# AnimatePortrait/AnimatePortrait

Measured on AMD Instinct MI355X. Metric: generator frames/sec @256x256 bs=16, higher is better.
Workload: dtype f32 (fp32 tensors; wide convs multiply fp32-class on the bf16 pipe: operands as bf16 head + tail, 3 products of 16-bit significands per multiply, ~2^-17 relative per product, fp32 accumulate); 1 GPU; Module2 generator resnet_9blocks_rcatland32_full_ifw fwd-only, ngf=64, bs=16/GPU, 256x256, fp32 (BASELINE configs[1]); global_batch=16, parallelism=dp1 (frame batches sharded, no collective), weights=random init N(0,0.02), seed 1234

## Files before the change

### animateportrait_amd/autograd.py

```python
import collections

import torch

from . import ops
from .ops import Feat, ConvSpec, ACT_NONE, ACT_RELU, ACT_LRELU, ACT_TANH, PAD_ZERO, PAD_REFLECT, W_OIHW, W_IOHW


_DIRECT = 0


class direct_param_grads:

    def __enter__(self):
        global _DIRECT
        _DIRECT += 1

    def __exit__(self, *exc):
        global _DIRECT
        _DIRECT -= 1
        return False


class Tape:
    def __init__(self):
# ... 159 lines not shown

def conv_backward(tape, layer, srcs, out, norm, act):
    contribs = tape.take(out)
    if not contribs:
        return
    plan = _backward_plan(tape, layer, srcs, out, norm, act, contribs)
    gfeat, gt, strip, db = _backward_norm(tape, plan, layer, out, act, contribs)
    _backward_weight(tape, plan, layer, srcs, gfeat, gt)
    _backward_bias(tape, layer, norm, gfeat, db)
    _backward_data(tape, plan, layer, srcs, gfeat, strip)


def _backward_norm(tape, plan, layer, out, act, contribs):
    if plan.norm_route == 'split':
        return ops.instnorm_bwd_split(ops._split_contribs(contribs), out, plan.gt_dims, plan.want_xs, plan.want_strip) + (None,)
    if out.data.dtype != torch.float32:
        out = Feat(out.data.float(), out._mean, out._rstd, out.act)
        contribs = [(g.float() if g.dtype != torch.float32 else g, pd) for g, pd in contribs]
    db = None
    if plan.norm_route == 'instnorm':
        dy = ops.instnorm_bwd(contribs, out, out_bf16=plan.dy16)
    elif plan.norm_route == 'act_bias':
        dy, db = ops.act_bwd_bias(contribs, out.data, act, tape.slot(layer.bias))
    else:
        dy = ops.act_bwd(contribs, out.data, act)
    gfeat = Feat(dy)
    if plan.wgrad_operand == 'g_xs_presplit':
        ops.presplit(gfeat, layer.spec.precision)
    return gfeat, None, None, db


def _backward_weight(tape, plan, layer, srcs, gfeat, gt):
    if plan.wgrad_route is None:
        return
    s = layer.spec
    if s.transposed:
        dw = ops.wgrad(s.k, 2, s.pad, PAD_ZERO, srcs[0], [gfeat], layer.weight.shape, precision=s.precision,
                       out=tape.slot(layer.weight), route=plan.wgrad_route)
    else:
        g_xs = gfeat.xs if plan.wgrad_operand in ('g_xs_from_split', 'g_xs_presplit') else None
        dw = ops.wgrad(s.k, s.stride, s.pad, s.pad_mode, gfeat, srcs, layer.weight.shape, precision=s.precision,
                       out=tape.slot(layer.weight), g_t=gt, g_xs=g_xs, route=plan.wgrad_route)
    tape.add_param(layer.weight, dw)


def _backward_bias(tape, layer, norm, gfeat, db):
    if not layer.bias.requires_grad:
        return
    slot = tape.slot(layer.bias)
    if norm:
        tape.add_param(layer.bias, slot if slot is not None else torch.zeros_like(layer.bias))
    else:
        tape.add_param(layer.bias, db if db is not None else ops.bias_grad(gfeat.data, out=slot))


def _backward_data(tape, plan, layer, srcs, gfeat, strip):
    s = layer.spec
    c0 = 0
    for i, (f, c, route) in enumerate(zip(srcs, s.cin_segments, plan.dgrad)):
        if route is not None and route[0] == 'final_k7':
            tape.add(f, ops.final_dgrad_k7(gfeat, layer.weight), route[1])
        elif route is not None and route[0] == 'head':
            tape.add(f, ops.head_dgrad(gfeat, layer.weight, f.data.shape[2], f.data.shape[3]), route[1])
        elif route is not None:
            spec, _ = _dgrad_spec(layer, c)
            w = layer.weight.detach()
            if len(srcs) > 1:
                w = w[c0:c0 + c] if s.transposed else w[:, c0:c0 + c]
            packed = layer.packed_dgrad(i, spec, w)
            if route[0] == 'strip':
                packed_t = layer.packed_dgrad((i, 'T'), spec, w.transpose(2, 3))
                g = ops.conv2d_dgrad_strip(spec, gfeat, packed, packed_t, strip, out_bf16=f.data.dtype == torch.bfloat16)
            else:
                g = ops.conv2d(spec, [gfeat], packed, None).data
            tape.add(f, g, route[1])
        c0 += c


def conv_forward(tape, layer, srcs, norm_act=None, act=ACT_NONE, out_octet=False, raw16=False):
    if not isinstance(srcs, (list, tuple)):
        srcs = [srcs]
    raw16 = (raw16 and tape is not None and norm_act is not None and ops.BF16_RAW and ops.DEFAULT_PRECISION == ops.PRECISION_BF16 and
             layer.spec.precision == ops.PRECISION_BF16)
    out = layer.run(srcs, norm_act=norm_act, act=act, out_octet=out_octet and tape is None, out_bf16=raw16)
    if tape is not None:
        tape.track(out)
        norm = norm_act is not None
        tape.steps.append(lambda: conv_backward(tape, layer, srcs, out, norm, act))
    return out


def _reduced(tape, f):
    contribs = tape.take(f)
    if not contribs:
        return None
    g1, pad, g2 = ops._split_contribs(contribs)
    return g1 if (pad == 0 and g2 is None) else ops.fold_add(g1, pad, g2)


def materialize_forward(tape, f, residual=None, consumer=None):
    keep = tape is not None or (consumer is not None and not consumer.stages_split(f.data.shape))
    out = ops.materialize(f, residual=residual, keep_fp32=keep)
    if tape is not None:
        tape.track(out)

        def bwd():
            g = _reduced(tape, out)
            if g is None:
                return
            tape.add(f, g, 0)
            if residual is not None:
                tape.add(residual, g, 0)
        tape.steps.append(bwd)
    return out


def warp_forward(tape, f, motion, flow, ifmask, level, consumer=None):
    n, _, h, w = f.data.shape
    emit_xs = consumer is not None and ops.takes_split(consumer.spec, n, h, w)
    s2d = emit_xs and len(consumer.spec.cin_segments) == 1 and ops.s2d_eligible(consumer.spec, h, w)
    out = ops.warp_concat(f, motion, flow, ifmask, level, emit_xs=emit_xs, keep_fp32=tape is not None or not emit_xs, s2d=s2d)
    if tape is not None:
        tape.track(out)

        def bwd():
            g = _reduced(tape, out)
            if g is None or not tape.tracked(f):
                return
            tape.add(f, ops.warp_concat_bwd(g, motion, flow, ifmask, level), 0)
        tape.steps.append(bwd)
    return out


def batch_split_forward(tape, f, b):
    l1, l2 = f.batch_slice(0, b), f.batch_slice(b, 2 * b)
    if tape is not None:
        tape.track(l1)
        tape.track(l2)

        def bwd():
            tape.add(f, torch.cat([_reduced(tape, l1), _reduced(tape, l2)], 0), 0)
        tape.steps.append(bwd)
    return l1, l2


def _weights_stamp(params):
    return tuple(ops.weight_key(p) for p in params)


class _NetFn(torch.autograd.Function):
    @staticmethod
    def forward(ctx, net, n_inputs, input_needs_grad, *tensors):
        inputs, params = tensors[:n_inputs], tensors[n_inputs:]
        tape = Tape()
        with torch.no_grad():
            out = net._run(tape, input_needs_grad, *inputs)
        ctx.tape, ctx.net, ctx.out_feat = tape, net, out
        ctx.n_inputs, ctx.params = n_inputs, params
        ctx.stamp = _weights_stamp(params)
        ctx.in_feat = getattr(net, '_last_input_feat', None)
        return out.data

    @staticmethod
    def backward(ctx, gout):
        tape = ctx.tape
        if tape is None:
            raise RuntimeError('animateportrait_amd: backward through this network a second time: the layer tape is '
# ... 34 lines not shown
```

### animateportrait_amd/networks.py

```python
import functools

import torch
import torch.nn as nn
from torch.optim import lr_scheduler

from . import ops
from .autograd import (conv_forward, materialize_forward, warp_forward, batch_split_forward,
                       generator_apply, discriminator_apply)
from .ops import (Feat, ConvSpec, ACT_NONE, ACT_RELU, ACT_LRELU, ACT_TANH, PAD_ZERO, PAD_REFLECT,
                  W_OIHW, W_IOHW)

GENERATOR_NAMES = ('resnet_9blocks_rcatland32_full_ifw', 'resnet_style2_9blocks')
_REFERENCE_ONLY_G = (
    'resnet_9blocks', 'resnet_9blocks_rcatland', 'resnet_9blocks_rcatland3',
    'resnet_9blocks_rcatland32', 'resnet_10blocks_rcatland32', 'resnet_9blocks_rcatland4',
    'resnet_9blocks_rcatland32_fw', 'resnet_9blocks_rcatland32_fw2', 'resnet_9blocks_rcatland32_ifw',
    'resnet_9blocks_rcatland32_ifw_single2', 'resnet_9blocks_rcatland32_full_ifw_colorcoded',
    'resnet_9blocks_rcatland32_full_ifw2', 'resnet_9blocks_rcatland32_full_ifw_single',
    'resnet_9blocks_rcatland32_full_ifw_single2', 'resnet_9blocks_rcatland32_full_ifw_single3', 'regressor',
    'combiner', 'resnet_9blocks_rcatland2', 'resnet_6blocks', 'unet_128', 'unet_256')


class ConvLayer(nn.Module):

    def __init__(self, cin_segments, cout, k, stride=1, pad=0, pad_mode=PAD_ZERO, transposed=False,
                 output_padding=0):
        super().__init__()
        cin = sum(cin_segments)
        shape = (cin, cout, k, k) if transposed else (cout, cin, k, k)
        self.weight = nn.Parameter(torch.empty(shape, dtype=torch.float32))
        self.bias = nn.Parameter(torch.zeros(cout, dtype=torch.float32))
        self.spec = ConvSpec(cin_segments, cout, k, stride, pad, pad_mode, transposed, output_padding,
                             W_IOHW if transposed else W_OIHW)
        self._slots = {}
        self._rows_spec = None
        self._s2d_spec = None

    def _packed(self, slot_id, spec, view):
        slot = ops.packed_slot(spec, self.weight, view, self._slots.get(slot_id))
        self._slots[slot_id] = slot
        return slot.buf

    def packed_dgrad(self, seg, spec, view):
        return self._packed(('dgrad', seg), spec, ops.WeightView(view))

    def packed(self):
        return self._packed('fwd', self.spec, ops.WeightView(self.weight.detach()))

    def run(self, srcs, norm_act=None, act=ACT_NONE, out_octet=False, out_bf16=False):
        if not isinstance(srcs, (list, tuple)):
            srcs = [srcs]
        spec, packed = self.spec, None
        if norm_act is None and ops.conv_d0_ok(spec, srcs, act):
            return ops.conv_d0(srcs[0], self.weight, self.bias.detach(), act)
        if ops.stem_rows_eligible(spec) and not srcs[0].is_split_only:
            spec, packed = self.rows_spec(), self.packed_rows()
            srcs = [ops.presplit_rows(srcs[0], self.spec.k, self.spec.pad, self.spec.pad_mode)]
        elif (srcs[0].s2d is not None or not srcs[0].is_split_only) and ops.s2d_eligible(spec, *srcs[0].data.shape[2:]):
            spec, packed = self.s2d_spec(), self.packed_s2d()
            if srcs[0].s2d is None:
                srcs[0].s2d = ops.presplit_s2d(srcs[0])
            srcs = [srcs[0].s2d]
        if packed is None:
            packed = self.packed()
        if norm_act is None:
            return ops.conv2d(spec, srcs, packed, self.bias.detach(), act=act, out_octet=out_octet)
        return ops.conv2d(spec, srcs, packed, None, want_stats=True, out_act=norm_act, out_octet=out_octet,
                          out_bf16=out_bf16 and spec is self.spec)

    def stages_split(self, shape):
        n, _, h, w = shape
        if ops.stem_rows_eligible(self.spec) or ops.s2d_eligible(self.spec, h, w):
            return False
        return ops.takes_split(self.spec, n, h, w)

    def s2d_spec(self):
        if self._s2d_spec is None:
            self._s2d_spec = ops.s2d_spec(self.spec)
        return self._s2d_spec

    def packed_s2d(self):
        return self._packed('s2d', self.s2d_spec(), ops.WeightView(self.weight.detach(), s2d_c=self.spec.cin_segments[0]))

    def rows_spec(self):
        if self._rows_spec is None:
            self._rows_spec = ops.stem_rows_spec(self.spec)
        return self._rows_spec

    def packed_rows(self):
        return self._packed('rows', self.rows_spec(), ops.WeightView(self.weight.detach(), rows_c=self.spec.cin_segments[0]))


def _seq(**children):
    return nn.ModuleDict({k.lstrip('_'): v for k, v in children.items()})


class ResnetBlock(nn.Module):

    def __init__(self, dim):
        super().__init__()
        self.conv_block = _seq(_1=ConvLayer([dim], dim, 3, 1, 1, PAD_REFLECT),
                               _5=ConvLayer([dim], dim, 3, 1, 1, PAD_REFLECT))

    def run(self, x, tape=None, consumer=None):
        c1, c5 = self.conv_block['1'], self.conv_block['5']
        dim = c1.spec.cout
        keep = consumer is not None and not consumer.stages_split(x.data.shape)
        y = conv_forward(tape, c1, x, norm_act=ACT_RELU, raw16=True, out_octet=tape is None and ops.trunk_octet_ok(dim))
        y = conv_forward(tape, c5, y, norm_act=ACT_NONE, raw16=True,
                         out_octet=tape is None and ops.trunk_octet_ok(dim, residual=x, keep_fp32=keep))
        return materialize_forward(tape, y, residual=x, consumer=consumer)


class ResnetBlock2(nn.Module):

    def __init__(self, segs, dim_out):
        super().__init__()
        self.conv_block = _seq(_1=ConvLayer(segs, dim_out, 3, 1, 1, PAD_REFLECT),
                               _5=ConvLayer([dim_out], dim_out, 3, 1, 1, PAD_REFLECT))
        self.shortcut = _seq(_0=ConvLayer(segs, dim_out, 3, 1, 1, PAD_ZERO))

    def run(self, srcs, tape=None, consumer=None):
        c1, c5, sc = self.conv_block['1'], self.conv_block['5'], self.shortcut['0']
        y = conv_forward(tape, c1, srcs, norm_act=ACT_RELU, raw16=True, out_octet=tape is None and ops.trunk_octet_ok(c1.spec.cout))
        y = conv_forward(tape, c5, y, norm_act=ACT_NONE, raw16=True)
        s = conv_forward(tape, sc, srcs, norm_act=ACT_NONE)
        return materialize_forward(tape, y, residual=s, consumer=consumer)


class ResnetConditionTriGenerator32_full_ifw(nn.Module):

    def __init__(self, input_nc, output_nc, ngf=64, norm='instance', use_dropout=False, n_blocks=9,
                 padding_type='reflect', div=3, disp=1):
        super().__init__()
        if norm != 'instance':
            raise NotImplementedError('normalization layer [%s] is not available on the HIP path' % norm)
        if use_dropout:
            raise NotImplementedError('dropout is not available on the HIP path (the model sets no_dropout)')
        if padding_type != 'reflect':
            raise NotImplementedError('padding [%s] is not implemented' % padding_type)
        assert n_blocks >= 0
        self.n_blocks, self.div, self.disp = n_blocks, div, disp
        self.input_nc, self.output_nc, self.ngf = input_nc, output_nc, ngf
        h = ngf // 2
        con_dim = 16
        dim = ngf * 4
        self.model_tri_merge = ConvLayer([ngf * 4, ngf * 4, ngf * 4], dim, 3, 1, 1)
        self.model_tri00 = _seq(_1=ConvLayer([input_nc], h, 7, 1, 3, PAD_REFLECT))
        self.model_tri01 = _seq(_0=ConvLayer([ngf], ngf * 2, 3, 2, 1))
        self.model_tri02 = _seq(_0=ConvLayer([ngf * 2], ngf * 4, 3, 2, 1))
        self.model_tri10 = _seq(_1=ConvLayer([input_nc], ngf, 7, 1, 3, PAD_REFLECT))
        self.model_tri11 = _seq(_0=ConvLayer([ngf], ngf, 3, 2, 1))
        self.model_tri12 = _seq(_0=ConvLayer([ngf * 2], ngf * 4, 3, 2, 1))
        self.model_tri20 = _seq(_1=ConvLayer([input_nc], ngf, 7, 1, 3, PAD_REFLECT))
        self.model_tri21 = _seq(_0=ConvLayer([ngf], ngf * 2, 3, 2, 1))
        self.model_tri22 = _seq(_0=ConvLayer([ngf * 2], ngf * 2, 3, 2, 1))
        blocks = {}
        for i in range(n_blocks):
            if (i + disp) % div == 0:
                blocks[str(i)] = ResnetBlock2([dim, con_dim, con_dim], dim)
            else:
                blocks[str(i)] = ResnetBlock(dim)
        self.model2 = nn.ModuleDict(blocks)
        self.model3 = _seq(_0=ConvLayer([ngf * 4], ngf * 2, 3, 2, 1, transposed=True, output_padding=1),
                           _3=ConvLayer([ngf * 2], ngf, 3, 2, 1, transposed=True, output_padding=1),
# ... 292 lines not shown
```

### animateportrait_amd/ops.py

```python
import collections
import ctypes
import os

import torch

from . import _capi as C
from ._capi import ACT_NONE, ACT_RELU, ACT_LRELU, ACT_TANH, PAD_ZERO, PAD_REFLECT, W_OIHW, W_IOHW

EPS = 1e-5

WEIGHTS_EPOCH = 0


def weight_key(w):
    owner = getattr(w, '_flat_owner', None)
    return (w._version, w.data_ptr(), WEIGHTS_EPOCH, owner.epoch if owner is not None else 0)

PRECISION_FP32, PRECISION_BF16X3, PRECISION_BF16 = 0, 1, 2
PRECISION_BY_NAME = {'fp32': PRECISION_FP32, 'bf16x3': PRECISION_BF16X3, 'bf16': PRECISION_BF16}
DEFAULT_PRECISION = PRECISION_BY_NAME.get(os.environ.get('APAMD_PRECISION', 'bf16x3'), PRECISION_BF16X3)


_LAST_STREAM = {}
_STREAM_FENCE = os.environ.get('APAMD_NO_STREAM_FENCE', '0') != '1'


def _stream():
    s = torch.cuda.current_stream()
    if _STREAM_FENCE:
        dev = s.device.index
        last = _LAST_STREAM.get(dev)
        if last is not None and last.cuda_stream != s.cuda_stream and not torch.cuda.is_current_stream_capturing():
            ev = torch.cuda.Event()
            ev.record(last)
            s.wait_event(ev)
        _LAST_STREAM[dev] = s
    return ctypes.c_void_p(s.cuda_stream)


def _ptr(t):
    return ctypes.c_void_p(t.data_ptr()) if t is not None else ctypes.c_void_p(0)


def _stand_in(shape, device):
    return torch.empty(1, dtype=torch.float32, device=device).expand(shape)


def _require_device(t, name, allow_bf16=False):
    if not t.is_cuda:
        raise RuntimeError('animateportrait_amd: %s must live on the MI355X (got a %s tensor); '
                           'this package has no CPU path' % (name, t.device))
    if not t.is_contiguous() or not (t.dtype == torch.float32 or (allow_bf16 and t.dtype == torch.bfloat16)):
        raise RuntimeError('animateportrait_amd: %s must be contiguous fp32%s (got %s)' % (name, ' or bf16' if allow_bf16 else '', t.dtype))


BF16_RAW = os.environ.get('APAMD_NO_BF16_RAW', '0') != '1'
XS_WGRAD = os.environ.get('APAMD_NO_XS_WGRAD', '0') != '1'
XS_DIRECT = XS_WGRAD and os.environ.get('APAMD_NO_XS_DIRECT', '0') != '1'


class Feat:
    __slots__ = ('data', '_mean', '_rstd', 'act', 'xs', 'pending', 'xs_rows', 'xs_heads_only', 's2d', 'oct')

    def __init__(self, data, mean=None, rstd=None, act=ACT_NONE, pending=None):
        self.data, self._mean, self._rstd, self.act = data, mean, rstd, act
        self.pending = pending
        self.xs = None
        self.xs_rows = None
        self.xs_heads_only = False
        self.s2d = None
        self.oct = None

    @property
    def shape(self):
        return self.data.shape

    @property
    def dtype(self):
        return self.data.dtype

    @classmethod
    def split_only(cls, shape, xs):
        f = cls(_stand_in(shape, xs.device))
        f.xs = xs
        return f

    @property
    def is_split_only(self):
        return ((self.xs is not None or self.s2d is not None or self.oct is not None) and self.data.stride(0) == 0 and
# ... 209 lines not shown
        buf = torch.empty(n, dtype=torch.float32, device=weight.device)
        slot = PackedSlot(buf, False)
        if owner is not None and weight.is_cuda:
            eb = lib.ap_conv2d_pack_entry_bytes()
            room = (ctypes.c_ubyte * (4 * eb))()
            cv = view.c_view(spec)
            cnt = C.check(lib.ap_conv2d_pack_entries(ctypes.byref(d), ctypes.byref(cv), _ptr(buf), room, 4), 'pack_entries')
            if cnt > 0:
                ps = getattr(owner, '_packset', None)
                if ps is None:
                    ps = owner._packset = PackSet()
                ps.register(slot, weight, bytes(room)[:cnt * eb], cnt)
                slot.batched, slot.owner = True, owner
    if slot.batched and slot.key is not None:
        owner._packset.refresh(weight.device)
    else:
        d = spec.desc(1, 64, 64)
        dense = view.dense()
        _require_device(dense, 'weight')
        C.check(lib.ap_conv2d_pack_weights(ctypes.byref(d), _ptr(dense), _ptr(slot.buf), _stream()), 'pack_weights')
        slot.key = key
    return slot


def _src_of(f, bf16_bit=False):
    s = C.ApSrc()
    s.data, s.C = f.data.data_ptr(), f.data.shape[1]
    s.act = f.act | (0x100 if bf16_bit and f.data.dtype == torch.bfloat16 else 0)
    if f.virtual:
        s.mean, s.rstd = f.mean.data_ptr(), f.rstd.data_ptr()
    return s


def presplit(f, precision=None):
    if f.xs is None:
        _norm_apply_split(f, None, want_y=False, want_xs=True)
    if precision == PRECISION_BF16X3 and f.xs_heads_only:
        raise RuntimeError('a split-bf16 (bf16x3) layer was handed a split copy written without its tail planes '
                           '(made while the package mode was plain bf16)')
    return f.xs


ROW_CHANNELS = 32


def stem_rows_eligible(spec):
    return (spec.precision != PRECISION_FP32 and spec.k == 7 and spec.stride == 1 and spec.pad == 3 and
            not spec.transposed and len(spec.cin_segments) == 1 and spec.cin_segments[0] <= 4 and spec.cout >= 32 and
            spec.w_layout == W_OIHW and not spec.w_flip)


def stem_rows_spec(spec):
    s = ConvSpec([ROW_CHANNELS], spec.cout, spec.k, 1, spec.pad, spec.pad_mode)
    s.kh = 1
    s.precision = spec.precision
    s.alg_macs = spec.cin_segments[0] * spec.k * spec.k
    return s


def stem_rows_weight(weight):
    co, c, k, _ = weight.shape
    w = weight.permute(0, 2, 1, 3).reshape(co, k * c, 1, k)
    out = torch.zeros((co, ROW_CHANNELS, 1, k), dtype=weight.dtype, device=weight.device)
    out[:, :k * c] = w
    return out


def presplit_rows(f, k, pad, pad_mode):
    key = (k, pad, pad_mode)
    if f.xs_rows is None:
        f.xs_rows = {}
    hit = f.xs_rows.get(key)
    if hit is None:
        x = f.data
        n, c, h, w = x.shape
        _require_device(x, 'stem input')
        s = _src_of(f)
        xs = _alloc_xs((n, ROW_CHANNELS, h, w), x.device)
        C.check(C.lib().ap_split_prepass_rows(ctypes.byref(s), n, h, w, k, pad, pad_mode, _ptr(xs), _stream()),
                'split_prepass_rows')
        hit = Feat.split_only((n, ROW_CHANNELS, h, w), xs)
        f.xs_rows[key] = hit
    return hit


def s2d_eligible(spec, h, w):
    k_ok = spec.k == 4 or (spec.k == 3 and spec.precision == PRECISION_BF16X3 and spec.cin_segments[0] % 16 == 0 and
                           not os.environ.get('APAMD_NO_S2D3'))
    return (spec.precision != PRECISION_FP32 and k_ok and spec.stride == 2 and spec.pad == 1 and
            spec.pad_mode == PAD_ZERO and not spec.transposed and len(spec.cin_segments) == 1 and
            spec.cin_segments[0] >= 32 and spec.cin_segments[0] % 8 == 0 and spec.cout >= 48 and h % 2 == 0 and
            w % 2 == 0 and spec.w_layout == W_OIHW and not spec.w_flip and not os.environ.get('APAMD_NO_S2D'))


def s2d_spec(spec):
    s = ConvSpec([4 * spec.cin_segments[0]], spec.cout, 2, 1, 0, PAD_ZERO)
    s.precision = spec.precision
    s.s2d_k = 3 if spec.k == 3 else 0
    return s


def s2d_weight(weight):
    co, c, k = weight.shape[:3]
    if k == 3:
        weight = torch.nn.functional.pad(weight, (0, 1, 0, 1))
    return weight.reshape(co, c, 2, 2, 2, 2).permute(0, 3, 5, 1, 2, 4).reshape(co, 4 * c, 2, 2).contiguous()


def presplit_s2d(f):
    x = f.data
    n, c, h, w = x.shape
    _require_device(x, 'space-to-depth source')
    s = _src_of(f)
    shape = (n, 4 * c, h // 2 + 1, w // 2 + 1)
    xs = _alloc_xs(shape, x.device)
    C.check(C.lib().ap_split_prepass_s2d(ctypes.byref(s), n, h, w, _ptr(xs), _stream()), 'split_prepass_s2d')
    return Feat.split_only(shape, xs)


def _alloc_xs(shape, device):
    nbytes = C.check(C.lib().ap_split_prepass_bytes(*shape), 'split_prepass_bytes')
    return torch.empty(nbytes, dtype=torch.uint8, device=device)


def _norm_apply_split(f, residual, want_y, want_xs, xs_relu=False):
    x = f.data
    n, c, h, w = x.shape
    oct_src = f.oct is not None
    if oct_src:
        if want_y or not want_xs or (residual is not None and not residual.is_split_only):
            raise RuntimeError('a channel-octet raw output is read as a split copy only (no fp32 result, no fp32 residual)')
        _require_device(f.oct, 'norm/split source')
    else:
        _require_device(x, 'norm/split source', allow_bf16=True)
    s = C.ApSrc()
    s.data, s.C, s.act = (f.oct if oct_src else x).data_ptr(), c, f.act
    partial, tiles, mo, ro = None, 0, None, None
    if f.pending is not None:
        partial, tiles = f.pending
        f._alloc_stats()
        mo, ro = f._mean, f._rstd
    elif f._mean is not None:
        s.mean, s.rstd = f._mean.data_ptr(), f._rstd.data_ptr()
    r = None
    res_flag = 0
    if residual is not None:
        if residual.act != ACT_NONE and residual.virtual:
            raise ValueError('a normalised residual cannot carry an activation')
        if residual.data.shape != x.shape:
            raise ValueError('residual shape mismatch')
        r = C.ApSrc()
        r.C, r.act = c, ACT_NONE
        if residual.is_split_only:
            if residual.xs is None or residual.xs_heads_only:
                raise RuntimeError('a split-only residual needs both planes of its split copy')
            r.data = residual.xs.data_ptr()
            res_flag = 4
        else:
            r.data = residual.data.data_ptr()
            if residual.virtual:
                r.mean, r.rstd = residual.mean.data_ptr(), residual.rstd.data_ptr()
    y = torch.empty(x.shape, dtype=torch.float32, device=x.device) if want_y else None
    xs = _alloc_xs(x.shape, x.device) if want_xs else None
    flags = ((1 if DEFAULT_PRECISION == PRECISION_BF16 else 0) | (2 if xs_relu else 0) | res_flag |
             (8 if (x.dtype == torch.bfloat16 and not oct_src) else 0) | (16 if oct_src else 0))
    C.check(C.lib().ap_norm_apply_split_ex(ctypes.byref(s), _ptr(partial), tiles, EPS, _ptr(mo), _ptr(ro),
# ... 659 lines not shown
```

Baseline: 2333 frames/s.

## Add fused streaming 7x7 reflect-pad stem conv kernel with register-resident weights

Adds a dedicated kernel for 7x7 stride-1 reflection-padded stem convolutions with 1-4 input channels. It reads the fp32 image directly, does the reflect padding and bf16 hi/lo split in shared memory, keeps the packed weights in registers, and runs a persistent grid that prefetches the next tile while computing the current one. Outputs include bias, activation and the per-tile norm statistics. This replaces the separate row pre-split pass and the generic implicit-GEMM path for forward-only runs, removing an extra global round trip. The cost is a new code path used only when no tape is active, plus zero-padded MFMA work because only 4 channels are filled against a 7-tap kernel.

Result: no change. 2355 frames/s (median of 6 runs) (+0.9%).

```diff
diff --git a/animateportrait_amd/_stemapi.py b/animateportrait_amd/_stemapi.py
--- /dev/null
+++ b/animateportrait_amd/_stemapi.py
@@ -0,0 +1,39 @@
+import ctypes
+import threading
+
+from . import _capi
+
+c_f32p = _capi.c_f32p
+_DESC = ctypes.POINTER(_capi.ApConvDesc)
+
+SIGNATURES = {
+    'ap_conv_stem_ok': (ctypes.c_int32, [_DESC]),
+    'ap_conv_stem_packed_floats': (ctypes.c_int64, [_DESC]),
+    'ap_conv_stem_stat_tiles': (ctypes.c_int32, [_DESC]),
+    'ap_conv_stem_pack': (ctypes.c_int, [_DESC, c_f32p, c_f32p, ctypes.c_void_p]),
+    'ap_conv_stem_fwd': (ctypes.c_int, [_DESC, c_f32p, c_f32p, c_f32p, c_f32p, ctypes.c_int32, ctypes.c_void_p]),
+}
+
+_lib = None
+_lock = threading.Lock()
+
+
+def lib():
+    global _lib
+    if _lib is None:
+        with _lock:
+            if _lib is None:
+                _capi.lib()
+                l = ctypes.CDLL(_capi.LIB_PATH)
+                for name, (res, args) in SIGNATURES.items():
+                    if not hasattr(l, name):
+                        raise RuntimeError('animateportrait_amd: %s is stale: it lacks %s. Rebuild it '
+                                           '(make -C animateportrait_amd/csrc)' % (_capi.LIB_PATH, name))
+                    fn = getattr(l, name)
+                    fn.restype = res
+                    fn.argtypes = args
+                _lib = l
+    return _lib
+
+
+check = _capi.check
diff --git a/animateportrait_amd/autograd.py b/animateportrait_amd/autograd.py
--- a/animateportrait_amd/autograd.py
+++ b/animateportrait_amd/autograd.py
@@ -265,7 +265,7 @@
         srcs = [srcs]
     raw16 = (raw16 and tape is not None and norm_act is not None and ops.BF16_RAW and ops.DEFAULT_PRECISION == ops.PRECISION_BF16 and
              layer.spec.precision == ops.PRECISION_BF16)
-    out = layer.run(srcs, norm_act=norm_act, act=act, out_octet=out_octet and tape is None, out_bf16=raw16)
+    out = layer.run(srcs, norm_act=norm_act, act=act, out_octet=out_octet and tape is None, out_bf16=raw16, stream_stem=tape is None)
     if tape is not None:
         tape.track(out)
         norm = norm_act is not None
diff --git a/animateportrait_amd/csrc/conv_stem.h b/animateportrait_amd/csrc/conv_stem.h
--- /dev/null
+++ b/animateportrait_amd/csrc/conv_stem.h
@@ -0,0 +1,236 @@
+#pragma once
+#include "conv_igemm.h"
+
+namespace apamd {
+
+typedef __bf16 stem_bf16x8 __attribute__((ext_vector_type(8)));
+typedef float stem_f32x16 __attribute__((ext_vector_type(16)));
+
+constexpr int kStemTH = 16, kStemTW = 32;
+constexpr int kStemRows = kStemTH + 6;
+constexpr int kStemPW = 40;
+constexpr int kStemSteps = 14;
+constexpr int kStemPackUint4 = kStemSteps * 2 * 64;
+
+struct StemParams {
+    const float* x;
+    const uint4* wp;
+    const float* bias;
+    float* y;
+    float* stats;
+    int N, Cin, H, W, Cout, act;
+    int tiles_x, tiles_y;
+};
+
+struct StemPackParams {
+    const float* w;
+    uint4* out;
+    int Cin, Cout;
+};
+
+__device__ __forceinline__ unsigned stem_pack2(__bf16 a, __bf16 b) {
+    return (unsigned)__builtin_bit_cast(unsigned short, a) | ((unsigned)__builtin_bit_cast(unsigned short, b) << 16);
+}
+
+__global__ __launch_bounds__(256) void stem_pack_kernel(const StemPackParams p) {
+    const int idx = blockIdx.x * 256 + threadIdx.x;
+    const int total = (p.Cout / 32) * kStemSteps * 64;
+    if (idx >= total) return;
+    const int lane = idx & 63, s = (idx >> 6) % kStemSteps, cot = (idx >> 6) / kStemSteps;
+    const int co = cot * 32 + (lane & 31), h = lane >> 5, ky = s >> 1, ch = s & 1;
+    __bf16 hi[8], lo[8];
+#pragma unroll
+    for (int j = 0; j < 8; ++j) {
+        const int kx = 4 * ch + 2 * h + (j >> 2), c = j & 3;
+        const float v = (kx < 7 && c < p.Cin) ? p.w[(((long long)co * p.Cin + c) * 7 + ky) * 7 + kx] : 0.f;
+        hi[j] = (__bf16)v;
+        lo[j] = (__bf16)(v - (float)hi[j]);
+    }
+    uint4* const o = p.out + ((long long)cot * kStemSteps + s) * 128 + lane;
+    o[0] = make_uint4(stem_pack2(hi[0], hi[1]), stem_pack2(hi[2], hi[3]), stem_pack2(hi[4], hi[5]), stem_pack2(hi[6], hi[7]));
+    o[64] = make_uint4(stem_pack2(lo[0], lo[1]), stem_pack2(lo[2], lo[3]), stem_pack2(lo[4], lo[5]), stem_pack2(lo[6], lo[7]));
+}
+
+__device__ __forceinline__ int stem_mirror(int v, int n) {
+    v = v < 0 ? -v : v;
+    v = v >= n ? 2 * n - 2 - v : v;
+    return v < 0 ? 0 : (v >= n ? n - 1 : v);
+}
+
+template <int WCO, bool OCT>
+__global__ __launch_bounds__(256, 2) void conv_stem_kernel(const StemParams p) {
+    constexpr int WPX = 4 / WCO, NT = kStemTH / WPX;
+    constexpr int SLOTS = kStemRows * kStemPW, IT = (SLOTS + 255) / 256;
+    __shared__ uint2 xs[2][kStemRows][kStemPW];
+    __shared__ float sred[WPX][32 * WCO][2];
+    const int tid = threadIdx.x, lane = tid & 63, wave = tid >> 6, l32 = lane & 31, half = lane >> 5;
+    const int wco = wave % WCO, wpx = wave / WCO;
+    const int ntiles = p.N * p.tiles_y * p.tiles_x;
+
+    uint4 wreg[kStemSteps][2];
+    {
+        const uint4* wsrc = p.wp + (long long)wco * kStemPackUint4 + lane;
+#pragma unroll
+        for (int s = 0; s < kStemSteps; ++s) {
+            wreg[s][0] = wsrc[s * 128];
+            wreg[s][1] = wsrc[s * 128 + 64];
+        }
+    }
+    const long long cs = (long long)p.H * p.W;
+    float v[IT][4];
+    auto fetch = [&](int t) __attribute__((always_inline)) {
+        const int ftx = t % p.tiles_x, fty = (t / p.tiles_x) % p.tiles_y, fn = t / (p.tiles_x * p.tiles_y);
+        const float* const xn = p.x + (long long)fn * p.Cin * cs;
+#pragma unroll
+        for (int it = 0; it < IT; ++it) {
+            const int i = it * 256 + tid, r = i / kStemPW, px = i - r * kStemPW;
+            const bool live = i < SLOTS && px < kStemTW + 6;
+            const long long off = (long long)stem_mirror(fty * kStemTH - 3 + r, p.H) * p.W + stem_mirror(ftx * kStemTW - 3 + px, p.W);
+#pragma unroll
+            for (int c = 0; c < 4; ++c) v[it][c] = (live && c < p.Cin) ? xn[c * cs + off] : 0.f;
+        }
+    };
+    const int co_base = wco * 32;
+    const bool want_stats = p.stats != nullptr;
+    const long long hw = cs;
+    float bias_l = 0.f;
+    if (!OCT && p.bias != nullptr) bias_l = p.bias[co_base + l32];
+
+    int tile = blockIdx.x;
+    if (tile < ntiles) fetch(tile);
+#pragma unroll 1
+    for (; tile < ntiles; tile += gridDim.x) {
+        const int tx = tile % p.tiles_x, ty = (tile / p.tiles_x) % p.tiles_y, n = tile / (p.tiles_x * p.tiles_y);
+        const int oy0 = ty * kStemTH, ox0 = tx * kStemTW;
+#pragma unroll
+        for (int it = 0; it < IT; ++it) {
+            const int i = it * 256 + tid, r = i / kStemPW, px = i - r * kStemPW;
+            if (i < SLOTS) {
+                __bf16 hi[4], lo[4];
+#pragma unroll
+                for (int c = 0; c < 4; ++c) {
+                    hi[c] = (__bf16)v[it][c];
+                    lo[c] = (__bf16)(v[it][c] - (float)hi[c]);
+                }
+                xs[0][r][px] = make_uint2(stem_pack2(hi[0], hi[1]), stem_pack2(hi[2], hi[3]));
+                xs[1][r][px] = make_uint2(stem_pack2(lo[0], lo[1]), stem_pack2(lo[2], lo[3]));
+            }
+        }
+        __syncthreads();
+        if (tile + (int)gridDim.x < ntiles) fetch(tile + gridDim.x);
+
+        float s_acc[OCT ? 16 : 1], q_acc[OCT ? 16 : 1];
+#pragma unroll
+        for (int i = 0; i < (OCT ? 16 : 1); ++i) { s_acc[i] = 0.f; q_acc[i] = 0.f; }
+#pragma unroll 1
+        for (int q = 0; q < NT; ++q) {
+            const int row = wpx * NT + q, oy = oy0 + row;
+            if (oy >= p.H) break;
+            stem_f32x16 acc;
+#pragma unroll
+            for (int i = 0; i < 16; ++i) acc[i] = 0.f;
+#pragma unroll
+            for (int s = 0; s < kStemSteps; ++s) {
+                const int ky = s >> 1, ch = s & 1;
+                const uint2* src0 = &xs[0][row + ky][l32 + 4 * ch + 2 * half];
+                const uint2* src1 = &xs[1][row + ky][l32 + 4 * ch + 2 * half];
+                const uint2 h0 = src0[0], h1 = src0[1], t0 = src1[0], t1 = src1[1];
+                const stem_bf16x8 xh = __builtin_bit_cast(stem_bf16x8, make_uint4(h0.x, h0.y, h1.x, h1.y));
+                const stem_bf16x8 xl = __builtin_bit_cast(stem_bf16x8, make_uint4(t0.x, t0.y, t1.x, t1.y));
+                const stem_bf16x8 wh = __builtin_bit_cast(stem_bf16x8, wreg[s][0]);
+                const stem_bf16x8 wl = __builtin_bit_cast(stem_bf16x8, wreg[s][1]);
+                if (OCT) {
+                    acc = __builtin_amdgcn_mfma_f32_32x32x16_bf16(wl, xh, acc, 0, 0, 0);
+                    acc = __builtin_amdgcn_mfma_f32_32x32x16_bf16(wh, xl, acc, 0, 0, 0);
+                    acc = __builtin_amdgcn_mfma_f32_32x32x16_bf16(wh, xh, acc, 0, 0, 0);
+                } else {
+                    acc = __builtin_amdgcn_mfma_f32_32x32x16_bf16(xh, wl, acc, 0, 0, 0);
+                    acc = __builtin_amdgcn_mfma_f32_32x32x16_bf16(xl, wh, acc, 0, 0, 0);
+                    acc = __builtin_amdgcn_mfma_f32_32x32x16_bf16(xh, wh, acc, 0, 0, 0);
+                }
+            }
+            if (OCT) {
+                const int ox = ox0 + l32;
+                const bool ok = ox < p.W;
+#pragma unroll
+                for (int g = 0; g < 4; ++g) {
+                    const int co = co_base + g * 8 + 4 * half;
+                    float vv[4];
+#pragma unroll
+                    for (int j = 0; j < 4; ++j) vv[j] = acc[g * 4 + j] + (p.bias != nullptr ? p.bias[co + j] : 0.f);
+                    if (ok) {
+#pragma unroll
+                        for (int j = 0; j < 4; ++j) {
+                            s_acc[g * 4 + j] += vv[j];
+                            q_acc[g * 4 + j] += vv[j] * vv[j];
+                        }
+                        float* const dst = p.y + (((long long)n * (p.Cout >> 3) + (co >> 3)) * hw + (long long)oy * p.W + ox) * 8 + (co & 7);
+                        *reinterpret_cast<float4*>(dst) =
+                            make_float4(apply_act(vv[0], p.act), apply_act(vv[1], p.act), apply_act(vv[2], p.act), apply_act(vv[3], p.act));
+                    }
+                }
+            } else {
+                float* const yrow = p.y + ((long long)n * p.Cout + co_base + l32) * hw + (long long)oy * p.W;
+                const bool vec = (p.W & 3) == 0;
+#pragma unroll
+                for (int g = 0; g < 4; ++g) {
+                    const int ox = ox0 + g * 8 + 4 * half;
+                    float vv[4];
+#pragma unroll
+                    for (int j = 0; j < 4; ++j) vv[j] = acc[g * 4 + j] + bias_l;
+                    if (vec && ox + 3 < p.W) {
+                        s_acc[0] += (vv[0] + vv[1]) + (vv[2] + vv[3]);
+                        q_acc[0] += (vv[0] * vv[0] + vv[1] * vv[1]) + (vv[2] * vv[2] + vv[3] * vv[3]);
+                        *reinterpret_cast<float4*>(yrow + ox) =
+                            make_float4(apply_act(vv[0], p.act), apply_act(vv[1], p.act), apply_act(vv[2], p.act), apply_act(vv[3], p.act));
+                    } else {
+#pragma unroll
+                        for (int j = 0; j < 4; ++j)
+                            if (ox + j < p.W) {
+                                s_acc[0] += vv[j];
+                                q_acc[0] += vv[j] * vv[j];
+                                yrow[ox + j] = apply_act(vv[j], p.act);
+                            }
+                    }
+                }
+            }
+        }
+        if (!want_stats) {
+        } else if (OCT) {
+#pragma unroll
+            for (int i = 0; i < 16; ++i) {
+                float s = s_acc[i], q2 = q_acc[i];
+#pragma unroll
+                for (int sh = 1; sh < 32; sh <<= 1) {
+                    s += __shfl_xor(s, sh, 64);
+                    q2 += __shfl_xor(q2, sh, 64);
+                }
+                if (l32 == 0) {
+                    const int c = co_base + (i & 3) + 8 * (i >> 2) + 4 * half;
+                    sred[wpx][c][0] = s;
+                    sred[wpx][c][1] = q2;
+                }
+            }
+        } else {
+            const float s = s_acc[0] + __shfl_xor(s_acc[0], 32, 64), q2 = q_acc[0] + __shfl_xor(q_acc[0], 32, 64);
+            if (half == 0) {
+                sred[wpx][co_base + l32][0] = s;
+                sred[wpx][co_base + l32][1] = q2;
+            }
+        }
+        __syncthreads();
+        if (want_stats && tid < 32 * WCO) {
+            float s = 0.f, q2 = 0.f;
+#pragma unroll
+            for (int w = 0; w < WPX; ++w) {
+                s += sred[w][tid][0];
+                q2 += sred[w][tid][1];
+            }
+            float* const d = p.stats + (((long long)n * p.Cout + tid) * ((long long)p.tiles_x * p.tiles_y) + ty * p.tiles_x + tx) * 2;
+            d[0] = s;
+            d[1] = q2;
+        }
+    }
+}
+
+}
diff --git a/animateportrait_amd/csrc/conv_stem.hip b/animateportrait_amd/csrc/conv_stem.hip
--- /dev/null
+++ b/animateportrait_amd/csrc/conv_stem.hip
@@ -0,0 +1,88 @@
+#include "common.h"
+#include "../../include/animateportrait_stem.h"
+#include "conv_stem.h"
+
+namespace apamd {
+
+static bool stem_desc_ok(const ap_conv_desc* d) {
+    return d && !d->transposed && d->KH == 7 && d->KW == 7 && d->stride == 1 && d->pad == 3 && d->pad_mode == AP_PAD_REFLECT &&
+           d->nsrc == 1 && d->src[0].C >= 1 && d->src[0].C <= 4 && (d->Cout == 32 || d->Cout == 64) &&
+           d->precision == AP_PRECISION_BF16X3 && d->w_layout == AP_W_OIHW && !d->w_flip && !d->presplit && d->N >= 1 &&
+           d->H > d->pad && d->W > d->pad;
+}
+
+static int stem_wg_per_cu(const void* kfn) {
+    static std::mutex mu;
+    static std::vector<std::pair<const void*, int>> seen;
+    std::lock_guard<std::mutex> lk(mu);
+    for (const auto& s : seen)
+        if (s.first == kfn) return s.second;
+    int n = 0;
+    if (hipOccupancyMaxActiveBlocksPerMultiprocessor(&n, kfn, 256, 0) != hipSuccess || n < 1) n = 2;
+    seen.push_back({kfn, n});
+    return n;
+}
+
+static int stem_refuse(const ap_conv_desc* d) {
+    if (stem_desc_ok(d)) return AP_OK;
+    return fail(AP_ERR_UNSUPPORTED, "conv_stem: built for 7x7 stride-1 reflection-pad-3 layers with 1..4 input and 32 or 64 output "
+                                    "channels in split-bf16 arithmetic (ap_conv_stem_ok)");
+}
+
+}
+
+using namespace apamd;
+
+extern "C" {
+
+int32_t ap_conv_stem_ok(const ap_conv_desc* d) { return stem_desc_ok(d) ? 1 : 0; }
+
+int64_t ap_conv_stem_packed_floats(const ap_conv_desc* d) {
+    const int rc = stem_refuse(d);
+    return rc ? rc : (int64_t)(d->Cout / 32) * kStemPackUint4 * 4;
+}
+
+int32_t ap_conv_stem_stat_tiles(const ap_conv_desc* d) {
+    const int rc = stem_refuse(d);
+    return rc ? rc : ((d->H + kStemTH - 1) / kStemTH) * ((d->W + kStemTW - 1) / kStemTW);
+}
+
+int ap_conv_stem_pack(const ap_conv_desc* d, const float* weight, float* packed, ap_stream_t stream) {
+    const int rc = stem_refuse(d);
+    if (rc) return rc;
+    if (!weight || !packed) return fail(AP_ERR_INVALID, "conv_stem_pack: null weight/packed pointer");
+    StemPackParams p;
+    p.w = weight; p.out = reinterpret_cast<uint4*>(packed); p.Cin = d->src[0].C; p.Cout = d->Cout;
+    const int total = (d->Cout / 32) * kStemSteps * 64;
+    hipLaunchKernelGGL(stem_pack_kernel, dim3((total + 255) / 256), dim3(256), 0, (hipStream_t)stream, p);
+    return check_launch("stem_pack_kernel");
+}
+
+int ap_conv_stem_fwd(const ap_conv_desc* d, const float* packed, const float* bias, float* y, float* stat_partials, int32_t octet,
+                     ap_stream_t stream) {
+    const int rc = stem_refuse(d);
+    if (rc) return rc;
+    if (!packed || !y || !d->src[0].data) return fail(AP_ERR_INVALID, "conv_stem_fwd: null packed/y/source pointer");
+    if (d->src[0].mean || d->src[0].rstd || d->src[0].act != AP_ACT_NONE)
+        return fail(AP_ERR_UNSUPPORTED, "conv_stem_fwd: the source is a plain image (no statistics, no activation)");
+    if (d->act < 0 || d->act > 3) return fail(AP_ERR_INVALID, "conv_stem_fwd: act %d", d->act);
+    if ((reinterpret_cast<uintptr_t>(y) | reinterpret_cast<uintptr_t>(packed)) & 15)
+        return fail(AP_ERR_INVALID, "conv_stem_fwd: y and packed must be 16-byte aligned");
+    StemParams p;
+    p.x = d->src[0].data; p.wp = reinterpret_cast<const uint4*>(packed); p.bias = bias; p.y = y; p.stats = stat_partials;
+    p.N = d->N; p.Cin = d->src[0].C; p.H = d->H; p.W = d->W; p.Cout = d->Cout; p.act = d->act;
+    p.tiles_x = (d->W + kStemTW - 1) / kStemTW; p.tiles_y = (d->H + kStemTH - 1) / kStemTH;
+    const long long ntiles = (long long)d->N * p.tiles_y * p.tiles_x;
+    if (ntiles > 0x7fffffffLL) return fail(AP_ERR_UNSUPPORTED, "conv_stem_fwd: grid too large");
+    const void* kfn = d->Cout == 32 ? (octet ? (const void*)&conv_stem_kernel<1, true> : (const void*)&conv_stem_kernel<1, false>)
+                                    : (octet ? (const void*)&conv_stem_kernel<2, true> : (const void*)&conv_stem_kernel<2, false>);
+    const long long slots = (long long)num_cus() * stem_wg_per_cu(kfn);
+    const long long per = (ntiles + slots - 1) / slots;
+    const dim3 grid((unsigned)((ntiles + per - 1) / per)), block(256);
+    void* args[] = {&p};
+    const hipError_t e = hipLaunchKernel(kfn, grid, block, args, 0, (hipStream_t)stream);
+    if (e != hipSuccess) return fail(AP_ERR_LAUNCH, "conv_stem_kernel launch: %s", hipGetErrorString(e));
+    return check_launch("conv_stem_kernel");
+}
+
+}
diff --git a/animateportrait_amd/networks.py b/animateportrait_amd/networks.py
--- a/animateportrait_amd/networks.py
+++ b/animateportrait_amd/networks.py
@@ -35,6 +35,7 @@
         self._slots = {}
         self._rows_spec = None
         self._s2d_spec = None
+        self._stem = None
 
     def _packed(self, slot_id, spec, view):
         slot = ops.packed_slot(spec, self.weight, view, self._slots.get(slot_id))
@@ -47,10 +48,14 @@
     def packed(self):
         return self._packed('fwd', self.spec, ops.WeightView(self.weight.detach()))
 
-    def run(self, srcs, norm_act=None, act=ACT_NONE, out_octet=False, out_bf16=False):
+    def run(self, srcs, norm_act=None, act=ACT_NONE, out_octet=False, out_bf16=False, stream_stem=False):
         if not isinstance(srcs, (list, tuple)):
             srcs = [srcs]
         spec, packed = self.spec, None
+        if stream_stem and len(srcs) == 1 and ops.stem_stream_eligible(spec, srcs[0]):
+            if norm_act is None:
+                return ops.conv_stem(spec, srcs[0], self.packed_stem(), self.bias.detach(), act=act, out_octet=out_octet)
+            return ops.conv_stem(spec, srcs[0], self.packed_stem(), None, want_stats=True, out_act=norm_act, out_octet=out_octet)
         if norm_act is None and ops.conv_d0_ok(spec, srcs, act):
             return ops.conv_d0(srcs[0], self.weight, self.bias.detach(), act)
         if ops.stem_rows_eligible(spec) and not srcs[0].is_split_only:
@@ -81,6 +86,12 @@
 
     def packed_s2d(self):
         return self._packed('s2d', self.s2d_spec(), ops.WeightView(self.weight.detach(), s2d_c=self.spec.cin_segments[0]))
+
+    def packed_stem(self):
+        key = ops.weight_key(self.weight)
+        if self._stem is None or self._stem[0] != key or self._stem[1].device != self.weight.device:
+            self._stem = (key, ops.stem_pack(self.spec, self.weight.detach().contiguous()))
+        return self._stem[1]
 
     def rows_spec(self):
         if self._rows_spec is None:
diff --git a/animateportrait_amd/ops.py b/animateportrait_amd/ops.py
--- a/animateportrait_amd/ops.py
+++ b/animateportrait_amd/ops.py
@@ -5,6 +5,7 @@
 import torch
 
 from . import _capi as C
+from . import _stemapi as S
 from ._capi import ACT_NONE, ACT_RELU, ACT_LRELU, ACT_TANH, PAD_ZERO, PAD_REFLECT, W_OIHW, W_IOHW
 
 EPS = 1e-5
@@ -380,6 +381,60 @@
         hit = Feat.split_only((n, ROW_CHANNELS, h, w), xs)
         f.xs_rows[key] = hit
     return hit
+
+
+STEM_STREAM = os.environ.get('APAMD_NO_STEM_STREAM', '0') != '1'
+
+
+def stem_stream_eligible(spec, src):
+    if (not STEM_STREAM or not stem_rows_eligible(spec) or src.virtual or src.is_split_only or
+            src.data.dtype != torch.float32):
+        return False
+    d = spec.desc(1, *src.data.shape[2:])
+    return S.lib().ap_conv_stem_ok(ctypes.byref(d)) == 1
+
+
+def stem_pack(spec, weight):
+    _require_device(weight, 'weight')
+    d = spec.desc(1, 64, 64)
+    n = C.check(S.lib().ap_conv_stem_packed_floats(ctypes.byref(d)), 'conv_stem_packed_floats')
+    packed = torch.empty(n, dtype=torch.float32, device=weight.device)
+    C.check(S.lib().ap_conv_stem_pack(ctypes.byref(d), _ptr(weight), _ptr(packed), _stream()), 'conv_stem_pack')
+    return packed
+
+
+def conv_stem(spec, src, packed, bias=None, act=ACT_NONE, want_stats=False, out_act=ACT_NONE, out_octet=False):
+    x = src.data
+    n, _, h, w = x.shape
+    _require_device(x, 'stem input')
+    d = spec.desc(n, h, w, [src], act)
+    lib = S.lib()
+    out_octet = bool(out_octet)
+    if out_octet:
+        y = torch.empty((n, spec.cout // 8, h * w, 8), dtype=torch.float32, device=x.device)
+    else:
+        y = torch.empty((n, spec.cout, h, w), dtype=torch.float32, device=x.device)
+    partial = None
+    if want_stats:
+        tiles = C.check(lib.ap_conv_stem_stat_tiles(ctypes.byref(d)), 'conv_stem_stat_tiles')
+        partial = torch.empty((n * spec.cout, tiles, 2), dtype=torch.float32, device=x.device)
+    if PROFILER is not None:
+        e0, e1 = torch.cuda.Event(enable_timing=True), torch.cuda.Event(enable_timing=True)
+        e0.record()
+    C.check(lib.ap_conv_stem_fwd(ctypes.byref(d), _ptr(packed), _ptr(bias), _ptr(y), _ptr(partial), int(out_octet), _stream()),
+            'conv_stem_fwd')
+    if PROFILER is not None:
+        e1.record()
+        PROFILER.records.append(('conv_stem<%d%s>' % (spec.cout // 32, ', octet' if out_octet else ''),
+                                 2.0 * n * h * w * spec.cout * sum(spec.cin_segments) * spec.k ** 2, e0, e1))
+    if out_octet:
+        res = Feat(_stand_in((n, spec.cout, h, w), x.device), act=out_act if want_stats else ACT_NONE,
+                   pending=(partial, tiles) if want_stats else None)
+        res.oct = y
+        return res
+    if not want_stats:
+        return Feat(y)
+    return Feat(y, act=out_act, pending=(partial, tiles))
 
 
 def s2d_eligible(spec, h, w):
diff --git a/include/animateportrait_stem.h b/include/animateportrait_stem.h
--- /dev/null
+++ b/include/animateportrait_stem.h
@@ -0,0 +1,21 @@
+#ifndef ANIMATEPORTRAIT_STEM_H
+#define ANIMATEPORTRAIT_STEM_H
+
+#include "animateportrait_amd.h"
+
+#ifdef __cplusplus
+extern "C" {
+#endif
+
+int32_t ap_conv_stem_ok(const ap_conv_desc* d);
+int64_t ap_conv_stem_packed_floats(const ap_conv_desc* d);
+int32_t ap_conv_stem_stat_tiles(const ap_conv_desc* d);
+int ap_conv_stem_pack(const ap_conv_desc* d, const float* weight, float* packed, ap_stream_t stream);
+int ap_conv_stem_fwd(const ap_conv_desc* d, const float* packed, const float* bias, float* y, float* stat_partials, int32_t octet,
+                     ap_stream_t stream);
+
+#ifdef __cplusplus
+}
+#endif
+
+#endif
```
